# IONIQ6000/av1-go

Measured on AMD Instinct MI355X. Metric: encoded 4K30 frames/sec (whole node) at fixed QP; PSNR-Y delta vs libaom, higher is better.
Workload: dtype u16

## Files before the change

av1-go_amd/csrc/av1_entropy_kernels.hip:

```cpp
#include <stdlib.h>
#include <string.h>
#include <vector>
#include "av1_ops_cdfs.hpp"
#include "av1_ops8.hpp"
#include "av1mi_internal.hpp"
#include "chains_rank.hpp"

namespace av1mi {
using namespace av1ops;

struct Av1EntLaunch {
  FrameView fv;
  int nframes, sbr_n, sbc_n;
  BlockInfo *info;
  op_t *ops; uint32_t ops_cap;
  uint32_t *grouped; uint32_t grouped_cap;
  uint32_t *list_off, *grouped_off;
  uint32_t *cursors;
  uint16_t *slot_total, *slot_base;
  uint16_t *rec;
  uint32_t *nops;
  uint8_t *slots; uint32_t slot_cap;
  uint32_t *tile_size;
  uint64_t *group_sum;
// ... 42 lines not shown
  const long nb = (long)L.fv.w8 * L.fv.h8, i = (long)blockIdx.x * 256 + threadIdx.x;
  if (i >= nb * L.nframes) return;
  const int f = (int)(i / nb), b = (int)(i - (long)f * nb);
  const FrameView v = frame_view<0>(L, f);
  BlockInfo o = {};
  inter_mode_decision(v, b / v.w8, b % v.w8, &o);
  L.info[nb * f + b] = o;
}

struct TileWave {
  template <class T> using Var = LaneVar<T, 1>;
  template <class F> __device__ __forceinline__ void each(F f) { f((int)threadIdx.x); __syncthreads(); }
  __device__ __forceinline__ int scan(Var<int> &v) {
    const int lane = (int)threadIdx.x, x = v.v[0];
    int inc = x;
#pragma unroll
    for (int d = 1; d < 64; d <<= 1) {
      const int y = __shfl_up(inc, d, 64);
      if (lane >= d) inc += y;
    }
    v.v[0] = inc - x;
    return __shfl(inc, 63, 64);
  }
  __device__ __forceinline__ int first(Var<int> &v) { return __shfl(v.v[0], 0, 64); }
  __device__ __forceinline__ uint64_t ballot(Var<int> &v) { return __ballot(v.v[0] != 0); }
};

__global__ __launch_bounds__(64) __attribute__((amdgpu_waves_per_eu(2, 8))) void k_av1_tokens(Av1EntLaunch L) {
  const int tiles = L.sbr_n * L.sbc_n, t = blockIdx.x, f = t / tiles, tt = t - f * tiles, sbr = tt / L.sbc_n, sbc = tt - sbr * L.sbc_n;
  if (sbr < L.sb_rows32) return;
  const FrameView v = frame_view(L, f);
  __shared__ Tile8Mem S;
  const int below = tiles - L.sb_rows32 * L.sbc_n;
  uint16_t *rec = L.rec + ((size_t)f * below + (tt - (tiles - below))) * kBlocksPerTile * kBlockRecords;
  TileWave w;
  PoolAreas out = { L, (size_t)t };
  const int n = tok_tile8(w, S, v, sbr, sbc, rec, L.ops_cap, out);
  if (threadIdx.x == 0) {
    if (n < 0) atomicOr(L.status, 1u);
    L.nops[t] = n < 0 ? 0u : (uint32_t)n;
  }
}

__global__ __launch_bounds__(64) void k_av1_tokens32(Av1EntLaunch L) {
  __shared__ Tile32Mem S;
  const int tiles = L.sbr_n * L.sbc_n, band = L.sb_rows32 * L.sbc_n, f = blockIdx.x / band, tt = blockIdx.x - f * band, sbr = tt / L.sbc_n, sbc = tt - sbr * L.sbc_n;
  const size_t t = (size_t)f * tiles + tt;
  const FrameView v = frame_view<1>(L, f);
  TileWave w;
  PoolAreas out = { L, t };
  const int n = tok_tile32(w, S, v, sbr, sbc, L.ops_cap, out);
  if (threadIdx.x == 0) {
    if (n < 0) atomicOr(L.status, 1u);
    L.nops[t] = n < 0 ? 0u : (uint32_t)n;
  }
}

enum { kChainsInter = 0, kChainsKey8 = 1, kChainsKey32 = 2 };
enum { kChainsCapLds = 0, kChainsCapTickets = 1 };
constexpr int kChainsStaticLds = 64 * 16 * 2, kCuLds = 160 << 10, kChainsXcds = 8, kChainsCusPerXcd = 32;
constexpr int kChainsDefaultCap = kChainsCapTickets, kChainsDefaultWaves = 2;
constexpr int kTicketStride = 32, kTicketRowFirst = kTicketStride, kTicketRowBand32 = kTicketRowFirst + kChainsXcds * kTicketStride;
static unsigned chains_dynamic_lds(int waves) { return waves > 0 && kCuLds / waves > kChainsStaticLds ? (unsigned)(kCuLds / waves - kChainsStaticLds) : 0u; }

__device__ __forceinline__ void chains_item(const Av1EntLaunch &L, int ntiles_all, int flavour, int g, int k, uint16_t *s_big) {
  const int lane = threadIdx.x, t = g * 64 + lane;
  const int sl = (flavour == kChainsInter ? kChainsRankInter : flavour == kChainsKey8 ? kChainsRankKey8 : kChainsRankKey32)[k];
// ... 403 lines not shown
```

av1-go_amd/csrc/av1_ops.hpp:

```cpp
#pragma once
#include <stdint.h>

#if defined(__HIPCC__)
#include <hip/hip_runtime.h>
#define AV1_HD __host__ __device__ inline
#define AV1_UNROLL _Pragma("unroll")
#define AV1_NOUNROLL _Pragma("unroll 1")
#else
#define AV1_HD inline
#define AV1_UNROLL
#define AV1_NOUNROLL
#endif

namespace av1ops {

typedef uint16_t __attribute__((may_alias)) u16a;
typedef uint32_t __attribute__((may_alias)) u32a;
typedef uint64_t __attribute__((may_alias)) u64a;

enum Slot : int {
  S_SKIP = 0,
  S_PART8 = S_SKIP + 3,
  S_PART16 = S_PART8 + 1,
  S_PART32 = S_PART16 + 4,
// ... 46 lines not shown
  if (s == B.eob_y) return B.eob_y_n;
  if (s == B.eob_c) return B.eob_c_n;
  return s < B.base_eob_y ? 2 : s < B.base_y ? 3 : 4;
}
AV1_HD int slot_nsym(int s, bool key) {
  if (const int n = coeff_nsym<kSlots8>(s)) return n;
  if (s < S_PART8) return 2;
  if (s < S_PART16) return 4;
  if (s < S_USE_WIENER) return 10;
  if (s < S_COMMON_END) return 2;
  if (key) {
    if (s < S_UV_MODE) return 13;
    if (s < S_ANGLE) return 14;
    if (s < S_INTRA_TX) return 7;
    return 7;
  }
  if (s < S_MV_JOINT) return 2;
  if (s == S_MV_JOINT) return 4;
  if (s < S_INTER_TX) {
    const int k = (s - S_MV_COMP) & 15;
    return k == MVC_CLASS ? 11 : (k == MVC_CLASS0_FR || k == MVC_CLASS0_FR + 1 || k == MVC_FR) ? 4 : 2;
  }
  return 16;
}
AV1_HD int q_category(int base_q_idx) { return base_q_idx <= 20 ? 0 : base_q_idx <= 60 ? 1 : base_q_idx <= 120 ? 2 : 3; }
AV1_HD int slot_words(int nsym) { return nsym <= 4 ? 4 : nsym <= 8 ? 8 : 16; }

typedef uint32_t op_t;
struct SlotTable { uint16_t off[S_MAX]; uint8_t nsym[(S_MAX + 3) & ~3]; int words; };
AV1_HD op_t op_lit(int n, unsigned v) { return (op_t)(0x80000000u | ((unsigned)n << 27) | (v & 0x7FFu)); }
AV1_HD op_t make_tuple(uint32_t fl, uint32_t fh, int s, int n) { return (op_t)(((unsigned)(n - s) << 19) | ((fl >> 6) << 9) | (fh >> 6)); }
enum { kBlocksPerTile = 64, kSplitHorz = 14, kSplitVert = 15, kListAlign = 4, kBlockRecords = 1024 };

struct Sink {
  uint16_t *rec;
  uint8_t *cnt;
  int zi, nrec, n;
  bool overflow;
  AV1_HD void put(unsigned r) { if (nrec < kBlockRecords) rec[nrec] = (uint16_t)r; else overflow = true; nrec++; n++; }
  AV1_HD void sym(int slot, int s) {
    put(((unsigned)slot << 4) | (unsigned)s);
    uint8_t &c = cnt[slot * kBlocksPerTile + zi];
    if (c == 255) overflow = true; else c++;
  }
  AV1_HD void split(int kind, int slot) { sym(slot, kind ? kSplitVert : kSplitHorz); }
  AV1_HD void lit(unsigned v, int nbits) {
    while (nbits > 11) { nbits -= 11; put(0x8000u | (11u << 11) | ((v >> nbits) & 0x7FFu)); }
    if (nbits > 0) put(0x8000u | ((unsigned)nbits << 11) | (v & ((1u << nbits) - 1u)));
  }
};
struct BlockInfo { uint8_t mode, flags, num, drl; int16_t px, py; };
struct FrameView {
  int w8, h8;
  int key;
  const uint8_t *y_mode, *uv_mode;
  const int16_t *mv;
  const uint8_t *skip;
  const int16_t *lev_y, *lev_u, *lev_v;
  const BlockInfo *info;
  int lr_on[3];
  int8_t lr_unit[2][8];
  int lr_rows[3], lr_cols[3];
  const int8_t *lr_units[3];
  int cdef_bits;
  const uint8_t *cdef_idx;
};
AV1_HD unsigned cdef_index(const FrameView &f, int sbr, int sbc) { return f.cdef_idx ? f.cdef_idx[sbr * ((f.w8 + 7) / 8) + sbc] : 0u; }

AV1_HD int iabs(int v) { return v < 0 ? -v : v; }
AV1_HD int imin(int a, int b) { return a < b ? a : b; }
AV1_HD int imax(int a, int b) { return a > b ? a : b; }
AV1_HD int ilog2(unsigned v) { return 31 - __builtin_clz(v | 1u); }
// ... 543 lines not shown
```

av1-go_amd/csrc/av1_ops8.hpp:

```cpp
#pragma once
#include "av1_ops32.hpp"

namespace av1ops {

enum { kLanes8 = kBlocksPerTile, kReplaySlots = (S_MAX + 1) / 2, kOwn8 = (S_MAX + kLanes8 - 1) / kLanes8 };
static_assert(2 * kReplaySlots >= S_MAX && S_MAX <= 256 && kOwn8 * kLanes8 >= S_MAX && 4 * kLanes8 >= S_MAX, "rows are bytes; two passes cover every slot");

struct Tile8Mem {
  union {
    struct { uint8_t cnt[S_MAX * kBlocksPerTile]; alignas(16) uint8_t mag[kBlocksPerTile * kMagBytes]; } p1;
    uint16_t pos[kReplaySlots * kBlocksPerTile];
  };
  uint16_t total[S_MAX], base[S_MAX];
  uint8_t row[(S_MAX + 3) & ~3];
  uint8_t sums[kBlocksPerTile];
  ScanTables scan;
};
struct SlotCounts8 { uint32_t w[kOwn8][kBlocksPerTile / 4]; };

AV1_HD void replay_block8(const uint16_t *rec, int nrec, uint16_t *pos, const uint8_t *row, int blk, int first, op_t *list, uint32_t *grouped, int row_lo,
                          bool literals) {
  int n = first;
  for (int i0 = 0; i0 < nrec; i0 += 8) {
    struct alignas(16) R8 { uint32_t w[4]; } q = *reinterpret_cast<const R8 *>(rec + i0);
    AV1_UNROLL
    for (int j = 0; j < 8; j++, n++) {
      if (i0 + j >= nrec) break;
      const unsigned r = (q.w[j >> 1] >> (16 * (j & 1))) & 0xFFFFu;
      if (r & 0x8000u) { if (literals) list[n] = op_lit((int)((r >> 11) & 15), r & 0x7FFu); }
      else {
        const unsigned rw = (unsigned)row[r >> 4] - (unsigned)row_lo;
        if (rw < (unsigned)kReplaySlots) { uint16_t &p = pos[rw * kBlocksPerTile + blk]; grouped[p] = ((uint32_t)n << 4) | (r & 15u); p++; }
      }
    }
  }
}

template <class W, class O>
AV1_HD int tok_tile8(W &w, Tile8Mem &S, const FrameView &f, int sbr, int sbc, uint16_t *rec, uint32_t ops_cap, O &out) {
  typedef typename W::template Var<int> LaneInt;
  const int nslots = f.key ? S_KEY_END : S_INTER_END;
  w.each([&](int lane) {
    for (int i = lane; i < S_MAX * kBlocksPerTile / 4; i += kLanes8) reinterpret_cast<u32a *>(S.p1.cnt)[i] = 0;
    if (lane == 0) fill_scan_tables(&S.scan);
    int bx, by;
    demorton8((unsigned)lane, &bx, &by);
    const int r8 = sbr * 8 + by, c8 = sbc * 8 + bx;
    S.sums[by * 8 + bx] = (uint8_t)(r8 < f.h8 && c8 < f.w8 ? block_levels_summary(f, r8 * f.w8 + c8) : 0u);
  });
  int cdef_zi = -1;
  if (f.cdef_bits) {
    if (f.key) cdef_zi = 0;
    else {
      LaneInt coded;
      w.each([&](int lane) {
        int bx, by;
        demorton8((unsigned)lane, &bx, &by);
        const int r8 = sbr * 8 + by, c8 = sbc * 8 + bx;
        coded[lane] = r8 < f.h8 && c8 < f.w8 && !f.skip[r8 * f.w8 + c8];
      });
      const uint64_t m = w.ballot(coded);
      cdef_zi = m ? __builtin_ctzll(m) : -1;
    }
  }
  LaneInt nrec, first;
  w.each([&](int lane) {
    const TokScratch ts = { S.p1.mag + lane * kMagBytes, &S.scan };
    Sink k = { rec + (size_t)lane * kBlockRecords, S.p1.cnt, lane, 0, 0, false };
    tok_block(f, k, ts, sbr, sbc, lane, S.sums, cdef_zi);
    nrec[lane] = k.nrec;
    first[lane] = k.n | (k.overflow ? 1 << 24 : 0);
  });
  const int sum = w.scan(first), words = sum & 0xFFFFFF;
  bool fits = (uint32_t)words <= ops_cap && !(sum >> 24);
  typename W::template Var<SlotCounts8> cnt;
  if (fits) w.each([&](int lane) {
    SlotCounts8 &c = cnt[lane];
    AV1_UNROLL
    for (int q = 0; q < kOwn8; q++) {
      const int sl = lane + kLanes8 * q;
      int tot = 0;
      AV1_UNROLL
      for (int i = 0; i < kBlocksPerTile / 4; i++) {
        const uint32_t u = sl < nslots ? reinterpret_cast<const u32a *>(S.p1.cnt)[sl * (kBlocksPerTile / 4) + i] : 0u;
        c.w[q][i] = u;
#if defined(__HIP_DEVICE_COMPILE__)
        tot = (int)__builtin_amdgcn_sad_u8(u, 0u, (unsigned)tot);
#else
        tot += (int)((u & 0xFF) + ((u >> 8) & 0xFF) + ((u >> 16) & 0xFF) + (u >> 24));
#endif
      }
      if (sl < S_MAX) S.total[sl] = (uint16_t)tot;
    }
  });
  LaneInt ent, used;
  if (fits) w.each([&](int lane) {
    int e = 0, u = 0;
    for (int q = 0; q < 4; q++) {
      const int sl = 4 * lane + q;
      if (sl < nslots) { e += (S.total[sl] + kListAlign - 1) & ~(kListAlign - 1); u += S.total[sl] != 0; }
    }
// ... 14 lines not shown
    for (int q = 0; q < 4; q++) {
      const int sl = 4 * lane + q;
      if (sl >= nslots) break;
      const int tot = S.total[sl];
      S.base[sl] = (uint16_t)run; S.row[sl] = (uint8_t)r;
      run += (tot + kListAlign - 1) & ~(kListAlign - 1); r += tot != 0;
    }
  });
  const int npass = rows <= kReplaySlots ? 1 : 2;
  for (int pass = 0; pass < npass; pass++) {
    const int row_lo = pass * kReplaySlots;
    w.each([&](int lane) {
      const SlotCounts8 &c = cnt[lane];
      AV1_UNROLL
      for (int q = 0; q < kOwn8; q++) {
        const int sl = lane + kLanes8 * q;
        if (sl >= S_MAX) continue;
        if (pass == 0) { const bool on = sl < nslots; out.slot(sl, on ? S.total[sl] : (uint16_t)0, on ? S.base[sl] : (uint16_t)0); }
        if (sl >= nslots || !S.total[sl]) continue;
        const unsigned rw = (unsigned)S.row[sl] - (unsigned)row_lo;
        if (rw >= (unsigned)kReplaySlots) continue;
        int run = S.base[sl];
        AV1_UNROLL
        for (int i = 0; i < kBlocksPerTile / 4; i++) {
          const uint32_t u = c.w[q][i];
          const int p0 = run, p1 = p0 + (int)(u & 0xFF), p2 = p1 + (int)((u >> 8) & 0xFF), p3 = p2 + (int)((u >> 16) & 0xFF);
          run = p3 + (int)(u >> 24);
          u32a *d = reinterpret_cast<u32a *>(S.pos + rw * kBlocksPerTile + 4 * i);
          d[0] = (uint32_t)p0 | ((uint32_t)p1 << 16); d[1] = (uint32_t)p2 | ((uint32_t)p3 << 16);
        }
      }
    });
    w.each([&](int lane) {
      replay_block8(rec + (size_t)lane * kBlockRecords, nrec[lane], S.pos, S.row, lane, first[lane] & 0xFFFFFF, list, grouped, row_lo, pass == 0);
    });
  }
  return words;
}

}
```

av1-go_amd/host/av1_bitstream.hpp:

```cpp
#pragma once
#include <cstddef>
#include <cstdint>
#include <string>
#include <vector>

#include "../../include/av1mi_host.h"

namespace av1mi_host {
namespace av1 {

inline av1mi_colour unspecified_colour() { av1mi_colour c = {}; c.primaries = c.transfer = c.matrix = 2; return c; }
inline bool same_colour(const av1mi_colour &a, const av1mi_colour &b) {
  if (a.primaries != b.primaries || a.transfer != b.transfer || a.matrix != b.matrix || a.full_range != b.full_range || !a.have_mdcv != !b.have_mdcv || !a.have_cll != !b.have_cll) return false;
  if (a.have_cll && (a.max_cll != b.max_cll || a.max_fall != b.max_fall)) return false;
  if (!a.have_mdcv) return true;
  for (int i = 0; i < 3; i++) if (a.primary_x[i] != b.primary_x[i] || a.primary_y[i] != b.primary_y[i]) return false;
  return a.white_x == b.white_x && a.white_y == b.white_y && a.luminance_max == b.luminance_max && a.luminance_min == b.luminance_min;
}
struct SequenceParams {
  int width = 0, height = 0, bit_depth = 8;
  bool film_grain = false;
  av1mi_colour colour = unspecified_colour();
  bool described() const { return colour.primaries != 2 || colour.transfer != 2 || colour.matrix != 2; }
  bool has_colour() const { return described() || colour.full_range || colour.have_mdcv || colour.have_cll; }
  bool operator==(const SequenceParams &o) const {
    return width == o.width && height == o.height && bit_depth == o.bit_depth && film_grain == o.film_grain && same_colour(colour, o.colour);
  }
};
const char *colour_error(const av1mi_colour &c);

inline int visible_width(const av1mi_obu_frame &f) { return f.visible_width ? f.visible_width : f.width; }
inline int visible_height(const av1mi_obu_frame &f) { return f.visible_height ? f.visible_height : f.height; }
inline SequenceParams sequence_params(const av1mi_obu_frame &f) {
  SequenceParams sp; sp.width = visible_width(f); sp.height = visible_height(f); sp.bit_depth = f.bit_depth; sp.film_grain = f.film_grain_present != 0;
  if (f.colour) sp.colour = *f.colour;
  return sp;
}
std::vector<uint8_t> temporal_delimiter_obu();
std::vector<uint8_t> sequence_header_obu(const SequenceParams &sp);
std::vector<uint8_t> metadata_obu_hdr_cll(const av1mi_colour &c);
std::vector<uint8_t> metadata_obu_hdr_mdcv(const av1mi_colour &c);
void append_sequence_obus(const SequenceParams &sp, std::vector<uint8_t> *out);
bool frame_obu(const av1mi_obu_frame &f, int threads, std::vector<uint8_t> *out, std::string *err);
bool frame_obu_from_tiles(const av1mi_obu_frame &f, const uint8_t *payloads, const uint32_t *sizes, int ntiles, std::vector<uint8_t> *out,
                          std::string *err);
std::vector<uint8_t> range_code_raw(const uint32_t *fl, const uint32_t *fh, const uint8_t *sym, const uint8_t *nsym, size_t count);
bool opstream_supported(const av1mi_obu_frame &f, std::string *why);
bool opstream_tiles(const av1mi_obu_frame &f, std::vector<std::vector<uint8_t>> *tiles, std::string *err, int key_rows32 = 0);
int opstream_slots();
int opstream_tile32(const av1mi_obu_frame &f, int sbr, int sbc, uint32_t ops_cap, uint32_t *list, uint32_t *grouped, uint16_t *slot_total, uint16_t *slot_base,
                    std::string *err);
int opstream_tile8(const av1mi_obu_frame &f, int sbr, int sbc, uint32_t ops_cap, uint32_t *list, uint32_t *grouped, uint16_t *slot_total, uint16_t *slot_base,
                   std::string *err);
bool blocks_temporal_unit(const av1mi_obu_blocks &d, bool with_sequence_header, std::vector<uint8_t> *out, std::string *err, int threads = 1,
                          const size_t (*tile_start)[2] = nullptr);
bool temporal_unit(const av1mi_obu_frame &f, bool with_sequence_header, int threads, std::vector<uint8_t> *out, std::string *err);

}
}
```

av1-go_amd/host/av1_opstream.cpp:

```cpp
#include <algorithm>
#include <cstdio>
#include <cstdlib>
#include <cstring>
#include <string>
#include <vector>
#include "../csrc/av1_ops_cdfs.hpp"
#include "../csrc/av1_ops8.hpp"
#include "av1_bitstream.hpp"

namespace av1mi_host {
namespace av1 {

bool opstream_supported(const av1mi_obu_frame &f, std::string *why) {
  auto no = [&](const char *m) { if (why) *why = m; return false; };
  if (f.cdef_bits < 0 || f.cdef_bits > 3) return no("cdef_bits outside 0 .. 3");
  if (f.reduced_tx_set || f.disable_cdf_update) return no("reduced_tx_set / disable_cdf_update must be 0");
  if (f.tile_cols_log2 >= 0 || f.tile_rows_log2 >= 0) return no("one superblock per tile only");
  if (f.angle_y || f.angle_uv || f.cfl_alpha || f.tx_type || f.is_inter) return no("angle deltas, chroma from luma, transform types and intra blocks in inter frames are host-writer only");
  if (f.frame_type == 0 && f.skip) return no("key frames are coded with skip = 0");
  for (int p = 0; p < 3; p++) if (f.lr_type[p] > 1) return no("Wiener restoration only");
  if (f.lr_unit_shift || f.lr_uv_shift) return no("64x64 restoration units only");
  return true;
}

namespace {
bool code_list(std::vector<av1ops::op_t> &list, const std::vector<uint32_t> &grouped, int nslots, const uint16_t *total, const uint16_t *base,
               const av1ops::SlotTable &tab, const uint16_t *image, std::vector<uint8_t> *out, std::string *err) {
  using namespace av1ops;
  const int nops = (int)list.size();
  for (int sl = 0; sl < nslots; sl++)
    if (total[sl]) run_chain(&image[tab.off[sl]], tab.nsym[sl], &grouped[(size_t)base[sl]], total[sl], list.data());
  out->resize((size_t)nops * 2 + 64);
  Coder c;
  uint16_t stage[Coder::kStage];
  c.init(out->data(), (int)out->size(), stage);
  for (int i = 0; i < nops; i++) code_word(c, list[(size_t)i]);
  const int n = c.finish();
  if (n < 0) { if (err) *err = "tile payload overflow"; return false; }
  out->resize((size_t)n);
  return true;
}
struct WaveLoop {
  template <class T> using Var = av1ops::LaneVar<T, av1ops::kLanes32>;
  template <class F> void each(F f) { for (int lane = 0; lane < av1ops::kLanes32; lane++) f(lane); }
  int scan(Var<int> &v) {
    int run = 0;
    for (int lane = 0; lane < av1ops::kLanes32; lane++) { const int x = v.v[lane]; v.v[lane] = run; run += x; }
    return run;
  }
  int first(Var<int> &v) { return v.v[0]; }
  uint64_t ballot(Var<int> &v) {
    uint64_t m = 0;
    for (int lane = 0; lane < av1ops::kLanes32; lane++) m |= (uint64_t)(v.v[lane] != 0) << lane;
    return m;
  }
};
void frame_view_of(const av1mi_obu_frame &f, av1ops::FrameView *v) {
  memset(v, 0, sizeof(*v));
  v->w8 = f.width / 8; v->h8 = f.height / 8; v->key = f.frame_type == 0;
  v->y_mode = f.y_mode; v->uv_mode = f.uv_mode; v->mv = f.mv; v->skip = f.skip; v->lev_y = f.lev_y; v->lev_u = f.lev_u; v->lev_v = f.lev_v;
  v->cdef_bits = f.cdef_bits; v->cdef_idx = f.cdef_bits ? f.cdef_idx : nullptr;
  for (int p = 0; p < 3; p++) {
    v->lr_on[p] = f.lr_type[p] == 1;
    const int ph = p ? (visible_height(f) + 1) >> 1 : visible_height(f), pw = p ? (visible_width(f) + 1) >> 1 : visible_width(f);
    v->lr_rows[p] = std::max((ph + 32) / 64, 1); v->lr_cols[p] = std::max((pw + 32) / 64, 1);
  }
}
bool lr_units_of(const av1mi_obu_frame &f, av1ops::FrameView *v, std::string *err) {
  bool shared = true;
  for (int p = 0; p < 3; p++) {
    if (!v->lr_on[p]) continue;
    const int8_t *u = f.lr_units[p];
    const size_t n = (size_t)v->lr_rows[p] * v->lr_cols[p];
    for (size_t i = 0; i < n; i++) {
      if (u[i * 8] != 0 && u[i * 8] != 1) { if (err) *err = "Wiener restoration units only"; return false; }
      if (memcmp(u, u + i * 8, 8)) shared = false;
    }
    if (p == 2 && v->lr_on[1] && memcmp(u, f.lr_units[1], 8)) shared = false;
  }
  for (int p = 0; p < 3; p++) {
    if (!v->lr_on[p]) continue;
    if (shared) memcpy(v->lr_unit[p ? 1 : 0], f.lr_units[p], 8);
    else v->lr_units[p] = f.lr_units[p];
  }
  return true;
}
}

bool opstream_tiles(const av1mi_obu_frame &f, std::vector<std::vector<uint8_t>> *tiles, std::string *err, int key_rows32) {
  using namespace av1ops;
  if (!opstream_supported(f, err)) return false;
  if (key_rows32 && (f.frame_type != 0 || (key_rows32 & 63) || key_rows32 > f.height || (f.width & 31))) { if (err) *err = "bad 32x32 band"; return false; }
  FrameView v;
  frame_view_of(f, &v);
  std::vector<uint8_t> zskip;
  if (!v.key && !v.skip) { zskip.assign((size_t)v.w8 * v.h8, 0); v.skip = zskip.data(); }
  if (!lr_units_of(f, &v, err)) return false;
  const size_t nb = (size_t)v.w8 * v.h8;
  std::vector<BlockInfo> info(nb);
  v.info = info.data();
  for (size_t b = 0; b < nb; b++) memset(&info[b], 0, sizeof(BlockInfo));
  if (!v.key) for (int r = 0; r < v.h8; r++) for (int c = 0; c < v.w8; c++) inter_mode_decision(v, r, c, &info[(size_t)r * v.w8 + c]);
  const int qcat = q_category(f.base_q_idx);
  SlotTable tab;
  const std::vector<uint16_t> image = default_slot_image(v.key != 0, qcat, &tab);
  const int sbr_n = (v.h8 + 7) / 8, sbc_n = (v.w8 + 7) / 8;
  tiles->assign((size_t)sbr_n * sbc_n, {});
  const int nslots = v.key ? S_KEY_END : S_INTER_END;
  std::vector<Tile8Mem> mem8(1);
  std::vector<uint16_t> rec((size_t)kBlocksPerTile * kBlockRecords);
  const uint32_t ops_cap8 = 1u << 20;
  std::vector<op_t> list8(ops_cap8);
  std::vector<uint32_t> grouped8(65536 + kListAlign);
  const bool stats = getenv("AV1MI_TOK_STATS") != nullptr;
  int st_rec = 0, st_cnt = 0, st_ops = 0, st_over = 0; long st_ops_sum = 0;
  SlotTable tab32;
  const std::vector<uint16_t> image32 = key_rows32 ? default_slot_image_k32(qcat, &tab32) : std::vector<uint16_t>();
  std::vector<Tile32Mem> mem32(key_rows32 ? 1 : 0);
  const uint32_t ops_cap32 = 1u << 20;
  std::vector<op_t> list32(key_rows32 ? ops_cap32 : 0);
  std::vector<uint32_t> grouped32(key_rows32 ? 65536 : 0);
  for (int sbr = 0; sbr < sbr_n; sbr++)
    for (int sbc = 0; sbc < sbc_n; sbc++) {
      if (sbr * 64 < key_rows32) {
        WaveLoop wave;
        uint16_t base[S_MAX], total[S_MAX];
        CallerAreas out = { list32.data(), grouped32.data(), total, base };
        const int words = tok_tile32(wave, mem32[0], v, sbr, sbc, ops_cap32, out);
        if (words < 0) { if (err) *err = "tile too large for 16-bit entry positions"; return false; }
        std::vector<op_t> list(list32.begin(), list32.begin() + words);
        if (!code_list(list, grouped32, K_END, total, base, tab32, image32.data(), &(*tiles)[(size_t)sbr * sbc_n + sbc], err)) return false;
        continue;
      }
      WaveLoop wave;
      uint16_t base[S_MAX], total[S_MAX];
      CallerAreas out = { list8.data(), grouped8.data(), total, base };
      const int words = tok_tile8(wave, mem8[0], v, sbr, sbc, rec.data(), ops_cap8, out);
      if (stats) {
        std::vector<uint8_t> cnt((size_t)S_MAX * kBlocksPerTile, 0);
        const TokScratch ts = { mem8[0].p1.mag, &mem8[0].scan };
        int ops = 0;
        for (int zi = 0; zi < kBlocksPerTile; zi++) {
          Sink k = { rec.data(), cnt.data(), zi, 0, 0, false };
          tok_block(v, k, ts, sbr, sbc, zi, mem8[0].sums, -1);
          st_rec = std::max(st_rec, k.nrec); ops += k.n;
        }
        for (uint8_t c : cnt) st_cnt = std::max(st_cnt, (int)c);
        st_ops = std::max(st_ops, ops); st_ops_sum += ops;
        if (words < 0) { st_over++; continue; }
      }
      if (words < 0) { if (err) *err = "a tile exceeds the tokenizer's capacities (records or symbols of a slot per block, entries per tile)"; return false; }
      std::vector<op_t> list(list8.begin(), list8.begin() + words);
      if (!code_list(list, grouped8, nslots, total, base, tab, image.data(), &(*tiles)[(size_t)sbr * sbc_n + sbc], err)) return false;
    }
  if (stats)
    fprintf(stderr, "[av1mi tok stats] %d tiles: records per block <= %d (capacity %d), symbols of a slot in a block <= %d (255), list words per tile <= %d, mean %.0f; %d tiles over a block capacity\n",
            sbr_n * sbc_n, st_rec, (int)kBlockRecords, st_cnt, st_ops, (double)st_ops_sum / (sbr_n * sbc_n), st_over);
  return true;
}

int opstream_slots() { return av1ops::S_MAX; }

int opstream_tile8(const av1mi_obu_frame &f, int sbr, int sbc, uint32_t ops_cap, uint32_t *list, uint32_t *grouped, uint16_t *slot_total, uint16_t *slot_base,
                   std::string *err) {
  using namespace av1ops;
  if (!opstream_supported(f, err) || sbr < 0 || sbc < 0 || sbr * 64 >= f.height || sbc * 64 >= f.width) return -2;
  FrameView v;
  frame_view_of(f, &v);
  std::vector<uint8_t> zskip;
  if (!v.key && !v.skip) { zskip.assign((size_t)v.w8 * v.h8, 0); v.skip = zskip.data(); }
  if (!lr_units_of(f, &v, err)) return -2;
  std::vector<BlockInfo> info(v.key ? 0 : (size_t)v.w8 * v.h8);
  v.info = info.data();
  if (!v.key) for (int r = 0; r < v.h8; r++) for (int c = 0; c < v.w8; c++) { memset(&info[(size_t)r * v.w8 + c], 0, sizeof(BlockInfo)); inter_mode_decision(v, r, c, &info[(size_t)r * v.w8 + c]); }
  std::vector<Tile8Mem> mem(1);
  std::vector<uint16_t> rec((size_t)kBlocksPerTile * kBlockRecords);
  WaveLoop wave;
  CallerAreas out = { list, grouped, slot_total, slot_base };
  return tok_tile8(wave, mem[0], v, sbr, sbc, rec.data(), ops_cap, out);
}

int opstream_tile32(const av1mi_obu_frame &f, int sbr, int sbc, uint32_t ops_cap, uint32_t *list, uint32_t *grouped, uint16_t *slot_total, uint16_t *slot_base,
                    std::string *err) {
  using namespace av1ops;
  if (!opstream_supported(f, err) || f.frame_type != 0 || (f.width & 31) || sbr < 0 || sbc < 0 || (sbr + 1) * 64 > f.height || sbc * 64 >= f.width) return -2;
  FrameView v;
  frame_view_of(f, &v);
  if (!lr_units_of(f, &v, err)) return -2;
  std::vector<Tile32Mem> mem(1);
  WaveLoop wave;
  CallerAreas out = { list, grouped, slot_total, slot_base };
  return tok_tile32(wave, mem[0], v, sbr, sbc, ops_cap, out);
}

}
}
```

av1-go_amd/host/capi_host.cpp:

```cpp
#include <cstring>
#include "filmgrain.hpp"
#include "daemon.hpp"
#include "av1_bitstream.hpp"
#include "mux.hpp"
#include "y4m.hpp"
#include "backend.hpp"
#include "../csrc/quality.hpp"

using namespace av1mi_host;

static std::vector<std::string> split_lines(const std::string &s) {
  std::vector<std::string> a;
  size_t p = 0, q;
  while ((q = s.find('\n', p)) != std::string::npos) { a.push_back(s.substr(p, q - p)); p = q + 1; }
  a.push_back(s.substr(p));
  return a;
}

extern "C" {
int av1mi_host_determine_quality(int height) { return DetermineQuality(height); }
int av1mi_host_check_size_gate(long long orig, long long neu, double ratio) { return CheckSizeGate(orig, neu, ratio) ? 1 : 0; }
int av1mi_host_transcode_args(const char *in, const char *out, int has_video, int index, int height, int webrip, char *buf, int cap) {
  ProbeResult pr; pr.has_video_stream = has_video != 0; pr.VideoStream.Index = index; pr.VideoStream.Height = height;
  std::vector<std::string> a; std::string err;
// ... 290 lines not shown
  b.insert(b.end(), fr.begin(), fr.end());
  if ((long long)b.size() <= cap && out) memcpy(out, b.data(), b.size());
  return (long long)b.size();
}
long long av1mi_host_opstream_key32_temporal_unit(const av1mi_obu_frame *f, int key_rows32, int with_sequence_header, uint8_t *out, long long cap, char *err,
                                                  int errcap) {
  std::vector<std::vector<uint8_t>> tiles; std::string e;
  auto fail = [&](long long code) { if (err && errcap > 0) { strncpy(err, e.c_str(), errcap - 1); err[errcap - 1] = 0; } return code; };
  if (!av1::opstream_supported(*f, &e)) return fail(-2);
  if (!av1::opstream_tiles(*f, &tiles, &e, key_rows32)) return fail(-1);
  std::vector<uint8_t> cat; std::vector<uint32_t> sizes;
  for (auto &t : tiles) { sizes.push_back((uint32_t)t.size()); cat.insert(cat.end(), t.begin(), t.end()); }
  std::vector<uint8_t> fr;
  if (!av1::frame_obu_from_tiles(*f, cat.data(), sizes.data(), (int)sizes.size(), &fr, &e)) return fail(-1);
  std::vector<uint8_t> b = av1::temporal_delimiter_obu();
  if (with_sequence_header) av1::append_sequence_obus(av1::sequence_params(*f), &b);
  b.insert(b.end(), fr.begin(), fr.end());
  if ((long long)b.size() <= cap && out) memcpy(out, b.data(), b.size());
  return (long long)b.size();
}
int av1mi_host_opstream_slots(void) { return av1::opstream_slots(); }
int av1mi_host_opstream_tile32(const av1mi_obu_frame *f, int sbr, int sbc, uint32_t ops_cap, uint32_t *list, uint32_t *grouped, uint16_t *slot_total,
                               uint16_t *slot_base) {
  if (!f || !list || !grouped || !slot_total || !slot_base) return -2;
  std::string e;
  return av1::opstream_tile32(*f, sbr, sbc, ops_cap, list, grouped, slot_total, slot_base, &e);
}
int av1mi_host_opstream_tile8(const av1mi_obu_frame *f, int sbr, int sbc, uint32_t ops_cap, uint32_t *list, uint32_t *grouped, uint16_t *slot_total,
                              uint16_t *slot_base) {
  if (!f || !list || !grouped || !slot_total || !slot_base) return -2;
  std::string e;
  return av1::opstream_tile8(*f, sbr, sbc, ops_cap, list, grouped, slot_total, slot_base, &e);
}
long long av1mi_host_opstream_temporal_unit(const av1mi_obu_frame *f, int with_sequence_header, uint8_t *out, long long cap, char *err, int errcap) {
  return av1mi_host_opstream_key32_temporal_unit(f, 0, with_sequence_header, out, cap, err, errcap);
}
int av1mi_host_job_json(const char *id, const char *source, const char *status, const char *reason, long long orig, long long neu, char *buf, int cap) {
  Job j; j.ID = id; j.SourcePath = source; j.Status = status; j.Reason = reason; j.OriginalSize = orig; j.NewSize = neu; j.CreatedAt = "2026-01-02T03:04:05Z";
  const std::string s = JobToJSON(j);
  strncpy(buf, s.c_str(), cap - 1); buf[cap - 1] = 0;
  return (int)s.size();
}
double av1mi_host_gpu_usage(int device, const char *sysfs_root) { return GetGPUUsage(device, sysfs_root ? sysfs_root : "/sys"); }
int av1mi_host_mux_units(const char *path, int w, int h, int bd, int fps_n, int fps_d, const uint8_t *data, const long long *sizes,
                         const uint8_t *keys, int n) {
  return av1mi_host_mux_units_colour(path, w, h, bd, fps_n, fps_d, data, sizes, keys, n, nullptr);
}
int av1mi_host_mux_units_display(const char *path, int w, int h, int bd, int fps_n, int fps_d, const uint8_t *data, const long long *sizes,
                                 const uint8_t *keys, int n, int display_w, int display_h) {
  StreamSink sink; std::string err;
  av1::SequenceParams sp; sp.width = w; sp.height = h; sp.bit_depth = bd;
  if (display_w || display_h) sink.set_display_size(display_w, display_h);
  if (!sink.open(path, sp, fps_n, fps_d, &err)) return 1;
  for (int i = 0; i < n; i++) {
    std::vector<uint8_t> tu(data, data + sizes[i]);
    data += sizes[i];
    if (!sink.write(tu, keys[i] != 0, &err)) { sink.abort(); return 2; }
  }
  return sink.close(&err) ? 0 : 3;
}
int av1mi_host_job_pool(const char *sources, int workers, int ngpus, double ratio, const char *state_dir, char *buf, int cap) {
  std::vector<Job> jobs;
  for (const std::string &path : split_lines(sources)) {
    Job j; j.ID = "pool" + std::to_string(jobs.size()); j.SourcePath = path;
    FILE *f = fopen(path.c_str(), "rb");
    if (f) { fseek(f, 0, SEEK_END); j.OriginalSize = ftell(f); fclose(f); }
// ... 13 lines not shown
```

Before: 3482.

## Interleave per-block token records into lane-chunked rows with a compact front region

Replaces the per-block contiguous record buffer (1024 records per block) with a layout where records are stored in 8-record chunks interleaved across the 64 lanes, split into a front region of 12 rows per tile and a tail region stored separately for all tiles. The aim is to make the lanes' writes and the 16-byte replay reads adjacent across the wave, and to keep the commonly used first rows of all tiles packed together so they stay in cache. The cost is extra address arithmetic on every record write and read. Host stats and a self-test check the new layout against the old flat layout.

```diff
diff --git a/av1-go_amd/csrc/av1_entropy_kernels.hip b/av1-go_amd/csrc/av1_entropy_kernels.hip
--- a/av1-go_amd/csrc/av1_entropy_kernels.hip
+++ b/av1-go_amd/csrc/av1_entropy_kernels.hip
@@ -98,7 +98,7 @@
   const FrameView v = frame_view(L, f);
   __shared__ Tile8Mem S;
   const int below = tiles - L.sb_rows32 * L.sbc_n;
-  uint16_t *rec = L.rec + ((size_t)f * below + (tt - (tiles - below))) * kBlocksPerTile * kBlockRecords;
+  const TileRecords rec = TileRecords::of_tile(L.rec, (size_t)f * below + (tt - (tiles - below)), (size_t)L.nframes * below);
   TileWave w;
   PoolAreas out = { L, (size_t)t };
   const int n = tok_tile8(w, S, v, sbr, sbc, rec, L.ops_cap, out);
diff --git a/av1-go_amd/csrc/av1_ops.hpp b/av1-go_amd/csrc/av1_ops.hpp
--- a/av1-go_amd/csrc/av1_ops.hpp
+++ b/av1-go_amd/csrc/av1_ops.hpp
@@ -102,12 +102,28 @@
 AV1_HD op_t make_tuple(uint32_t fl, uint32_t fh, int s, int n) { return (op_t)(((unsigned)(n - s) << 19) | ((fl >> 6) << 9) | (fh >> 6)); }
 enum { kBlocksPerTile = 64, kSplitHorz = 14, kSplitVert = 15, kListAlign = 4, kBlockRecords = 1024 };
 
+enum { kRecChunk = 8, kRecRow = kBlocksPerTile * kRecChunk, kRecRows = kBlockRecords / kRecChunk, kFrontRows = 12, kTailRows = kRecRows - kFrontRows };
+static_assert(kRecRows * kRecChunk == kBlockRecords && kFrontRows > 0 && kFrontRows % 2 == 0 && kTailRows > 0, "whole chunks; a front and a tail");
+#ifdef AV1_TILE_RECORDS_OWN
+AV1_TILE_RECORDS_OWN
+#else
+struct TileRecords {
+  uint16_t *front, *tail;
+  AV1_HD uint16_t *at(int lane, int i) const {
+    const int row = i >> 3;
+    return (row < kFrontRows ? front + row * kRecRow : tail + (row - kFrontRows) * kRecRow) + lane * kRecChunk + (i & (kRecChunk - 1));
+  }
+  static AV1_HD TileRecords of_tile(uint16_t *base, size_t t, size_t tiles) {
+    return { base + t * ((size_t)kFrontRows * kRecRow), base + tiles * ((size_t)kFrontRows * kRecRow) + t * ((size_t)kTailRows * kRecRow) };
+  }
+};
+#endif
 struct Sink {
-  uint16_t *rec;
+  TileRecords rec;
   uint8_t *cnt;
   int zi, nrec, n;
   bool overflow;
-  AV1_HD void put(unsigned r) { if (nrec < kBlockRecords) rec[nrec] = (uint16_t)r; else overflow = true; nrec++; n++; }
+  AV1_HD void put(unsigned r) { if (nrec < kBlockRecords) *rec.at(zi, nrec) = (uint16_t)r; else overflow = true; nrec++; n++; }
   AV1_HD void sym(int slot, int s) {
     put(((unsigned)slot << 4) | (unsigned)s);
     uint8_t &c = cnt[slot * kBlocksPerTile + zi];
diff --git a/av1-go_amd/csrc/av1_ops8.hpp b/av1-go_amd/csrc/av1_ops8.hpp
--- a/av1-go_amd/csrc/av1_ops8.hpp
+++ b/av1-go_amd/csrc/av1_ops8.hpp
@@ -18,11 +18,11 @@
 };
 struct SlotCounts8 { uint32_t w[kOwn8][kBlocksPerTile / 4]; };
 
-AV1_HD void replay_block8(const uint16_t *rec, int nrec, uint16_t *pos, const uint8_t *row, int blk, int first, op_t *list, uint32_t *grouped, int row_lo,
+AV1_HD void replay_block8(const TileRecords &rec, int nrec, uint16_t *pos, const uint8_t *row, int blk, int first, op_t *list, uint32_t *grouped, int row_lo,
                           bool literals) {
   int n = first;
-  for (int i0 = 0; i0 < nrec; i0 += 8) {
-    struct alignas(16) R8 { uint32_t w[4]; } q = *reinterpret_cast<const R8 *>(rec + i0);
+  for (int i0 = 0; i0 < nrec; i0 += kRecChunk) {
+    struct alignas(16) R8 { uint32_t w[4]; } q = *reinterpret_cast<const R8 *>(rec.at(blk, i0));
     AV1_UNROLL
     for (int j = 0; j < 8; j++, n++) {
       if (i0 + j >= nrec) break;
@@ -37,7 +37,7 @@
 }
 
 template <class W, class O>
-AV1_HD int tok_tile8(W &w, Tile8Mem &S, const FrameView &f, int sbr, int sbc, uint16_t *rec, uint32_t ops_cap, O &out) {
+AV1_HD int tok_tile8(W &w, Tile8Mem &S, const FrameView &f, int sbr, int sbc, const TileRecords &rec, uint32_t ops_cap, O &out) {
   typedef typename W::template Var<int> LaneInt;
   const int nslots = f.key ? S_KEY_END : S_INTER_END;
   w.each([&](int lane) {
@@ -66,7 +66,7 @@
   LaneInt nrec, first;
   w.each([&](int lane) {
     const TokScratch ts = { S.p1.mag + lane * kMagBytes, &S.scan };
-    Sink k = { rec + (size_t)lane * kBlockRecords, S.p1.cnt, lane, 0, 0, false };
+    Sink k = { rec, S.p1.cnt, lane, 0, 0, false };
     tok_block(f, k, ts, sbr, sbc, lane, S.sums, cdef_zi);
     nrec[lane] = k.nrec;
     first[lane] = k.n | (k.overflow ? 1 << 24 : 0);
@@ -147,7 +147,7 @@
       }
     });
     w.each([&](int lane) {
-      replay_block8(rec + (size_t)lane * kBlockRecords, nrec[lane], S.pos, S.row, lane, first[lane] & 0xFFFFFF, list, grouped, row_lo, pass == 0);
+      replay_block8(rec, nrec[lane], S.pos, S.row, lane, first[lane] & 0xFFFFFF, list, grouped, row_lo, pass == 0);
     });
   }
   return words;
diff --git a/av1-go_amd/host/av1_bitstream.hpp b/av1-go_amd/host/av1_bitstream.hpp
--- a/av1-go_amd/host/av1_bitstream.hpp
+++ b/av1-go_amd/host/av1_bitstream.hpp
@@ -51,7 +51,7 @@
 int opstream_tile32(const av1mi_obu_frame &f, int sbr, int sbc, uint32_t ops_cap, uint32_t *list, uint32_t *grouped, uint16_t *slot_total, uint16_t *slot_base,
                     std::string *err);
 int opstream_tile8(const av1mi_obu_frame &f, int sbr, int sbc, uint32_t ops_cap, uint32_t *list, uint32_t *grouped, uint16_t *slot_total, uint16_t *slot_base,
-                   std::string *err);
+                   std::string *err, int32_t *block_records = nullptr);
 bool blocks_temporal_unit(const av1mi_obu_blocks &d, bool with_sequence_header, std::vector<uint8_t> *out, std::string *err, int threads = 1,
                           const size_t (*tile_start)[2] = nullptr);
 bool temporal_unit(const av1mi_obu_frame &f, bool with_sequence_header, int threads, std::vector<uint8_t> *out, std::string *err);
diff --git a/av1-go_amd/host/av1_opstream.cpp b/av1-go_amd/host/av1_opstream.cpp
--- a/av1-go_amd/host/av1_opstream.cpp
+++ b/av1-go_amd/host/av1_opstream.cpp
@@ -54,6 +54,10 @@
     for (int lane = 0; lane < av1ops::kLanes32; lane++) m |= (uint64_t)(v.v[lane] != 0) << lane;
     return m;
   }
+};
+struct OneTileRecords {
+  std::vector<uint16_t> front = std::vector<uint16_t>((size_t)av1ops::kFrontRows * av1ops::kRecRow), tail = std::vector<uint16_t>((size_t)av1ops::kTailRows * av1ops::kRecRow);
+  av1ops::TileRecords view() { return { front.data(), tail.data() }; }
 };
 void frame_view_of(const av1mi_obu_frame &f, av1ops::FrameView *v) {
   memset(v, 0, sizeof(*v));
@@ -108,12 +112,13 @@
   tiles->assign((size_t)sbr_n * sbc_n, {});
   const int nslots = v.key ? S_KEY_END : S_INTER_END;
   std::vector<Tile8Mem> mem8(1);
-  std::vector<uint16_t> rec((size_t)kBlocksPerTile * kBlockRecords);
+  OneTileRecords rec;
   const uint32_t ops_cap8 = 1u << 20;
   std::vector<op_t> list8(ops_cap8);
   std::vector<uint32_t> grouped8(65536 + kListAlign);
   const bool stats = getenv("AV1MI_TOK_STATS") != nullptr;
   int st_rec = 0, st_cnt = 0, st_ops = 0, st_over = 0; long st_ops_sum = 0;
+  std::vector<long> st_rows(kRecRows + 2, 0);
   SlotTable tab32;
   const std::vector<uint16_t> image32 = key_rows32 ? default_slot_image_k32(qcat, &tab32) : std::vector<uint16_t>();
   std::vector<Tile32Mem> mem32(key_rows32 ? 1 : 0);
@@ -135,15 +140,19 @@
       WaveLoop wave;
       uint16_t base[S_MAX], total[S_MAX];
       CallerAreas out = { list8.data(), grouped8.data(), total, base };
-      const int words = tok_tile8(wave, mem8[0], v, sbr, sbc, rec.data(), ops_cap8, out);
+      const int words = tok_tile8(wave, mem8[0], v, sbr, sbc, rec.view(), ops_cap8, out);
       if (stats) {
         std::vector<uint8_t> cnt((size_t)S_MAX * kBlocksPerTile, 0);
         const TokScratch ts = { mem8[0].p1.mag, &mem8[0].scan };
         int ops = 0;
         for (int zi = 0; zi < kBlocksPerTile; zi++) {
-          Sink k = { rec.data(), cnt.data(), zi, 0, 0, false };
+          int bx, by;
+          demorton8((unsigned)zi, &bx, &by);
+          if (sbr * 8 + by >= v.h8 || sbc * 8 + bx >= v.w8) continue;
+          Sink k = { rec.view(), cnt.data(), zi, 0, 0, false };
           tok_block(v, k, ts, sbr, sbc, zi, mem8[0].sums, -1);
           st_rec = std::max(st_rec, k.nrec); ops += k.n;
+          st_rows[std::min((k.nrec + kRecChunk - 1) / kRecChunk, (int)kRecRows + 1)]++;
         }
         for (uint8_t c : cnt) st_cnt = std::max(st_cnt, (int)c);
         st_ops = std::max(st_ops, ops); st_ops_sum += ops;
@@ -156,13 +165,18 @@
   if (stats)
     fprintf(stderr, "[av1mi tok stats] %d tiles: records per block <= %d (capacity %d), symbols of a slot in a block <= %d (255), list words per tile <= %d, mean %.0f; %d tiles over a block capacity\n",
             sbr_n * sbc_n, st_rec, (int)kBlockRecords, st_cnt, st_ops, (double)st_ops_sum / (sbr_n * sbc_n), st_over);
+  if (stats) {
+    fprintf(stderr, "[av1mi tok stats] blocks by record rows of %d (front = %d rows):", (int)kRecChunk, (int)kFrontRows);
+    for (size_t r = 0; r < st_rows.size(); r++) if (st_rows[r]) fprintf(stderr, " %zu:%ld", r, st_rows[r]);
+    fprintf(stderr, "\n");
+  }
   return true;
 }
 
 int opstream_slots() { return av1ops::S_MAX; }
 
 int opstream_tile8(const av1mi_obu_frame &f, int sbr, int sbc, uint32_t ops_cap, uint32_t *list, uint32_t *grouped, uint16_t *slot_total, uint16_t *slot_base,
-                   std::string *err) {
+                   std::string *err, int32_t *block_records) {
   using namespace av1ops;
   if (!opstream_supported(f, err) || sbr < 0 || sbc < 0 || sbr * 64 >= f.height || sbc * 64 >= f.width) return -2;
   FrameView v;
@@ -174,10 +188,20 @@
   v.info = info.data();
   if (!v.key) for (int r = 0; r < v.h8; r++) for (int c = 0; c < v.w8; c++) { memset(&info[(size_t)r * v.w8 + c], 0, sizeof(BlockInfo)); inter_mode_decision(v, r, c, &info[(size_t)r * v.w8 + c]); }
   std::vector<Tile8Mem> mem(1);
-  std::vector<uint16_t> rec((size_t)kBlocksPerTile * kBlockRecords);
+  OneTileRecords rec;
   WaveLoop wave;
   CallerAreas out = { list, grouped, slot_total, slot_base };
-  return tok_tile8(wave, mem[0], v, sbr, sbc, rec.data(), ops_cap, out);
+  const int words = tok_tile8(wave, mem[0], v, sbr, sbc, rec.view(), ops_cap, out);
+  if (block_records) {
+    std::vector<uint8_t> cnt((size_t)S_MAX * kBlocksPerTile, 0);
+    const TokScratch ts = { mem[0].p1.mag, &mem[0].scan };
+    for (int zi = 0; zi < kBlocksPerTile; zi++) {
+      Sink k = { rec.view(), cnt.data(), zi, 0, 0, false };
+      tok_block(v, k, ts, sbr, sbc, zi, mem[0].sums, -1);
+      block_records[zi] = k.nrec;
+    }
+  }
+  return words;
 }
 
 int opstream_tile32(const av1mi_obu_frame &f, int sbr, int sbc, uint32_t ops_cap, uint32_t *list, uint32_t *grouped, uint16_t *slot_total, uint16_t *slot_base,
diff --git a/av1-go_amd/host/capi_host.cpp b/av1-go_amd/host/capi_host.cpp
--- a/av1-go_amd/host/capi_host.cpp
+++ b/av1-go_amd/host/capi_host.cpp
@@ -346,6 +346,12 @@
   std::string e;
   return av1::opstream_tile8(*f, sbr, sbc, ops_cap, list, grouped, slot_total, slot_base, &e);
 }
+int av1mi_host_opstream_tile8_records(const av1mi_obu_frame *f, int sbr, int sbc, uint32_t ops_cap, uint32_t *list, uint32_t *grouped, uint16_t *slot_total,
+                                      uint16_t *slot_base, int32_t *block_records) {
+  if (!f || !list || !grouped || !slot_total || !slot_base || !block_records) return -2;
+  std::string e;
+  return av1::opstream_tile8(*f, sbr, sbc, ops_cap, list, grouped, slot_total, slot_base, &e, block_records);
+}
 long long av1mi_host_opstream_temporal_unit(const av1mi_obu_frame *f, int with_sequence_header, uint8_t *out, long long cap, char *err, int errcap) {
   return av1mi_host_opstream_key32_temporal_unit(f, 0, with_sequence_header, out, cap, err, errcap);
 }
diff --git a/av1-go_amd/host/records_selftest.cpp b/av1-go_amd/host/records_selftest.cpp
--- /dev/null
+++ b/av1-go_amd/host/records_selftest.cpp
@@ -0,0 +1,213 @@
+#include <stdint.h>
+#include <stdio.h>
+#include <string.h>
+#include <algorithm>
+#include <string>
+#include <vector>
+#include "av1_bitstream.hpp"
+#define AV1_TILE_RECORDS_OWN \
+  struct TileRecords { uint16_t *base; AV1_HD uint16_t *at(int lane, int i) const { return base + (size_t)lane * kBlockRecords + i; } };
+namespace records_selftest {
+#include "../csrc/av1_ops8.hpp"
+}
+
+namespace {
+namespace ops = records_selftest::av1ops;
+
+struct WaveLoop {
+  template <class T> using Var = ops::LaneVar<T, ops::kLanes32>;
+  template <class F> void each(F f) { for (int lane = 0; lane < ops::kLanes32; lane++) f(lane); }
+  int scan(Var<int> &v) {
+    int run = 0;
+    for (int lane = 0; lane < ops::kLanes32; lane++) { const int x = v.v[lane]; v.v[lane] = run; run += x; }
+    return run;
+  }
+  int first(Var<int> &v) { return v.v[0]; }
+  uint64_t ballot(Var<int> &v) {
+    uint64_t m = 0;
+    for (int lane = 0; lane < ops::kLanes32; lane++) m |= (uint64_t)(v.v[lane] != 0) << lane;
+    return m;
+  }
+};
+
+uint64_t rng_state = 1;
+uint32_t rnd() { rng_state ^= rng_state << 13; rng_state ^= rng_state >> 7; rng_state ^= rng_state << 17; return (uint32_t)(rng_state >> 16); }
+
+struct Frame {
+  int w, h, bd, q; bool key;
+  std::vector<uint8_t> y_mode, uv_mode, skip;
+  std::vector<int16_t> mv, lev_y, lev_u, lev_v;
+  Frame(int w_, int h_, int bd_, int q_, bool key_) : w(w_), h(h_), bd(bd_), q(q_), key(key_) {
+    const size_t nb = (size_t)(w / 8) * (h / 8);
+    y_mode.assign(nb, 0); uv_mode.assign(nb, 0); skip.assign(nb, 0); mv.assign(nb * 2, 0);
+    lev_y.assign(nb * 64, 0); lev_u.assign(nb * 16, 0); lev_v.assign(nb * 16, 0);
+  }
+  av1mi_obu_frame obu() const {
+    av1mi_obu_frame f;
+    memset(&f, 0, sizeof(f));
+    f.width = w; f.height = h; f.bit_depth = bd; f.frame_type = key ? 0 : 1; f.base_q_idx = q;
+    f.tile_cols_log2 = f.tile_rows_log2 = -1;
+    f.lev_y = lev_y.data(); f.lev_u = lev_u.data(); f.lev_v = lev_v.data();
+    if (key) { f.y_mode = y_mode.data(); f.uv_mode = uv_mode.data(); }
+    else { f.mv = mv.data(); f.skip = skip.data(); }
+    return f;
+  }
+  ops::FrameView view(std::vector<ops::BlockInfo> *info) const {
+    ops::FrameView v;
+    memset(&v, 0, sizeof(v));
+    v.w8 = w / 8; v.h8 = h / 8; v.key = key;
+    v.y_mode = y_mode.data(); v.uv_mode = uv_mode.data(); v.mv = mv.data(); v.skip = skip.data();
+    v.lev_y = lev_y.data(); v.lev_u = lev_u.data(); v.lev_v = lev_v.data();
+    for (int p = 0; p < 3; p++) { v.lr_rows[p] = std::max(((p ? (h + 1) / 2 : h) + 32) / 64, 1); v.lr_cols[p] = std::max(((p ? (w + 1) / 2 : w) + 32) / 64, 1); }
+    info->assign((size_t)v.w8 * v.h8, ops::BlockInfo());
+    for (ops::BlockInfo &b : *info) memset(&b, 0, sizeof(b));
+    v.info = info->data();
+    if (!key) for (int r = 0; r < v.h8; r++) for (int c = 0; c < v.w8; c++) ops::inter_mode_decision(v, r, c, &(*info)[(size_t)r * v.w8 + c]);
+    return v;
+  }
+  int block(int sbr, int sbc, int zi) const {
+    int bx, by;
+    ops::demorton8((unsigned)zi, &bx, &by);
+    const int r8 = sbr * 8 + by, c8 = sbc * 8 + bx;
+    return r8 < h / 8 && c8 < w / 8 ? r8 * (w / 8) + c8 : -1;
+  }
+};
+
+void count_records(const Frame &fr, int sbr, int sbc, int nrec[64]) {
+  std::vector<ops::BlockInfo> info;
+  const ops::FrameView v = fr.view(&info);
+  std::vector<ops::Tile8Mem> mem(1);
+  ops::Tile8Mem &S = mem[0];
+  memset(S.p1.cnt, 0, sizeof(S.p1.cnt));
+  ops::fill_scan_tables(&S.scan);
+  for (int zi = 0; zi < 64; zi++) {
+    int bx, by;
+    ops::demorton8((unsigned)zi, &bx, &by);
+    const int b = fr.block(sbr, sbc, zi);
+    S.sums[by * 8 + bx] = (uint8_t)(b >= 0 ? ops::block_levels_summary(v, b) : 0u);
+  }
+  static std::vector<uint16_t> flat((size_t)ops::kBlocksPerTile * ops::kBlockRecords);
+  for (int zi = 0; zi < 64; zi++) {
+    const ops::TokScratch ts = { S.p1.mag, &S.scan };
+    ops::Sink k = { { flat.data() }, S.p1.cnt, zi, 0, 0, false };
+    ops::tok_block(v, k, ts, sbr, sbc, zi, S.sums, -1);
+    nrec[zi] = k.nrec;
+  }
+}
+
+bool shape_block(Frame *fr, int zi, int target) {
+  static const int16_t kValues[] = { 0, 0, 1, -1, 2, 3, -6, 9, 14, -15, 40, -300, 2000, -30000 };
+  const int b = fr->block(0, 0, zi);
+  int nrec[64];
+  count_records(*fr, 0, 0, nrec);
+  for (int it = 0; it < 40000 && nrec[zi] != target; it++) {
+    if (it % 4000 == 3999) {
+      for (int i = 0; i < 64; i++) fr->lev_y[(size_t)b * 64 + i] = 0;
+      for (int i = 0; i < 16; i++) fr->lev_u[(size_t)b * 16 + i] = fr->lev_v[(size_t)b * 16 + i] = 0;
+      count_records(*fr, 0, 0, nrec);
+    }
+    const int p = (int)(rnd() % 96u);
+    int16_t *lev = p < 64 ? &fr->lev_y[(size_t)b * 64 + p] : p < 80 ? &fr->lev_u[(size_t)b * 16 + p - 64] : &fr->lev_v[(size_t)b * 16 + p - 80];
+    const int16_t old = *lev;
+    const int before = nrec[zi] > target ? nrec[zi] - target : target - nrec[zi];
+    *lev = kValues[rnd() % (sizeof(kValues) / sizeof(kValues[0]))];
+    count_records(*fr, 0, 0, nrec);
+    const int after = nrec[zi] > target ? nrec[zi] - target : target - nrec[zi];
+    if (after > before && !(after <= before + 6 && rnd() % 8u == 0)) { *lev = old; count_records(*fr, 0, 0, nrec); }
+  }
+  return nrec[zi] == target;
+}
+
+int failures = 0;
+#define CHECK(cond, ...) do { if (!(cond)) { failures++; fprintf(stderr, "records_selftest: " __VA_ARGS__); fprintf(stderr, "\n"); } } while (0)
+
+int compare_tile(const char *name, const Frame &fr, int sbr, int sbc, uint32_t ops_cap = 1u << 16) {
+  const int ns = ops::S_MAX;
+  const uint32_t fill32 = 0xA5A5A5A5u; const uint16_t fill16 = 0x5A5A;
+  std::vector<uint32_t> list_a(ops_cap, fill32), list_b(ops_cap, fill32), grp_a(ops_cap + 4 * ns, fill32), grp_b(ops_cap + 4 * ns, fill32);
+  std::vector<uint16_t> tot_a(ns, fill16), tot_b(ns, fill16), base_a(ns, fill16), base_b(ns, fill16);
+  const av1mi_obu_frame f = fr.obu();
+  std::string err;
+  const int na = av1mi_host::av1::opstream_tile8(f, sbr, sbc, ops_cap, list_a.data(), grp_a.data(), tot_a.data(), base_a.data(), &err);
+  std::vector<ops::BlockInfo> info;
+  const ops::FrameView v = fr.view(&info);
+  std::vector<ops::Tile8Mem> mem(1);
+  std::vector<uint16_t> flat((size_t)ops::kBlocksPerTile * ops::kBlockRecords);
+  WaveLoop wave;
+  ops::CallerAreas out = { list_b.data(), grp_b.data(), tot_b.data(), base_b.data() };
+  const int nb = ops::tok_tile8(wave, mem[0], v, sbr, sbc, ops::TileRecords{ flat.data() }, ops_cap, out);
+  CHECK(na == nb, "%s tile (%d, %d): %d list words, the plain layout gives %d (%s)", name, sbr, sbc, na, nb, err.c_str());
+  CHECK(list_a == list_b, "%s tile (%d, %d): list words differ", name, sbr, sbc);
+  CHECK(grp_a == grp_b, "%s tile (%d, %d): grouped entries differ", name, sbr, sbc);
+  CHECK(tot_a == tot_b && base_a == base_b, "%s tile (%d, %d): slot totals or bases differ", name, sbr, sbc);
+  if (na < 0) {
+    CHECK(std::all_of(tot_a.begin(), tot_a.end(), [](uint16_t t) { return t == 0; }), "%s: a refused tile keeps a slot total", name);
+    CHECK(std::all_of(list_a.begin(), list_a.end(), [&](uint32_t x) { return x == fill32; }) && std::all_of(grp_a.begin(), grp_a.end(), [&](uint32_t x) { return x == fill32; }),
+          "%s: a refused tile wrote list words or entries", name);
+  }
+  return na;
+}
+
+void noise(Frame *fr, int amplitude, unsigned share_of_256) {
+  auto one = [&](std::vector<int16_t> &lev) { for (int16_t &x : lev) x = rnd() % 256u < share_of_256 ? (int16_t)((int)(rnd() % (2u * amplitude + 1)) - amplitude) : 0; };
+  one(fr->lev_y); one(fr->lev_u); one(fr->lev_v);
+  for (uint8_t &m : fr->y_mode) m = (uint8_t)(rnd() % 13u);
+  for (uint8_t &m : fr->uv_mode) m = (uint8_t)(rnd() % 13u);
+  for (size_t i = 0; i < fr->skip.size(); i++) {
+    fr->skip[i] = rnd() % 4u == 0;
+    fr->mv[2 * i] = (int16_t)(2 * ((int)(rnd() % 41u) - 20)); fr->mv[2 * i + 1] = (int16_t)(2 * ((int)(rnd() % 41u) - 20));
+  }
+}
+}
+
+int main() {
+  const int F = 8 * ops::kFrontRows;
+  for (int key = 1; key >= 0; key--) {
+    Frame fr(64, 64, 8, 60, key != 0);
+    if (!key) for (uint8_t &s : fr.skip) s = 1;
+    {
+      const int b = fr.block(0, 0, 63);
+      if (!key) fr.skip[(size_t)b] = 0;
+      for (int i = 0; i < 64; i++) fr.lev_y[(size_t)b * 64 + i] = -32767;
+      for (int i = 0; i < 16; i++) { fr.lev_u[(size_t)b * 16 + i] = 32767; fr.lev_v[(size_t)b * 16 + i] = -32767; }
+    }
+    int longest[64];
+    count_records(fr, 0, 0, longest);
+    fprintf(stderr, "records_selftest: the longest block leaves %d records (capacity %d)\n", longest[63], (int)ops::kBlockRecords);
+    CHECK(longest[63] > 8 * (ops::kRecRows - 16) && longest[63] <= ops::kBlockRecords, "the longest block: %d records", longest[63]);
+    const int targets[] = { F - 1, F, F + 1, 2 * F + 5, 8 * 64 - 1, 8 * 100 };
+    const int blocks[] = { 20, 21, 22, 40, 61, 62 };
+    for (size_t i = 0; i < sizeof(targets) / sizeof(targets[0]); i++) {
+      if (!key) fr.skip[(size_t)fr.block(0, 0, blocks[i])] = 0;
+      CHECK(shape_block(&fr, blocks[i], targets[i]), "no block of %d records found (%s)", targets[i], key ? "key" : "inter");
+    }
+    int nrec[64];
+    count_records(fr, 0, 0, nrec);
+    fprintf(stderr, "records_selftest: %s tile, records per block:", key ? "key" : "inter");
+    for (int zi = 0; zi < 64; zi++) fprintf(stderr, " %d", nrec[zi]);
+    fprintf(stderr, "\n");
+    for (int want : { 7, 8, 9 })
+      if (key) CHECK(std::find(nrec, nrec + 64, want) != nrec + 64, "no block of %d records in the key tile", want);
+    const int words = compare_tile(key ? "boundaries, key" : "boundaries, inter", fr, 0, 0);
+    CHECK(words > 0, "the tile of boundary counts was refused");
+    CHECK(compare_tile("one word over the list's capacity", fr, 0, 0, (uint32_t)words - 1) == -1, "a tile over the list's capacity was not refused");
+    CHECK(compare_tile("exactly the list's capacity", fr, 0, 0, (uint32_t)words) == words, "a tile of exactly the list's capacity was refused");
+  }
+  const struct { int amplitude; unsigned share; } kNoise[] = { { 2, 20 }, { 40, 200 }, { 30000, 256 } };
+  for (int key = 1; key >= 0; key--)
+    for (const auto &nz : kNoise)
+      for (int bd = 8; bd <= 10; bd += 2) {
+        Frame fr(136, 72, bd, nz.amplitude > 100 ? 1 : 128, key != 0);
+        noise(&fr, nz.amplitude, nz.share);
+        for (int sbr = 0; sbr < 2; sbr++) for (int sbc = 0; sbc < 3; sbc++) {
+          const int n = compare_tile("noise", fr, sbr, sbc, 1u << 17);
+          CHECK(n > 0, "a tile of noise was refused");
+        }
+        int edge[64];
+        count_records(fr, 1, 2, edge);
+        CHECK(edge[0] > 0 && std::count(edge, edge + 64, 0) == 63, "the corner tile's blocks outside the frame leave records");
+      }
+  if (failures) { fprintf(stderr, "records_selftest: %d FAILURES\n", failures); return 1; }
+  printf("records_selftest OK (front %d rows, tail %d rows of %d records per lane)\n", (int)ops::kFrontRows, (int)ops::kTailRows, (int)ops::kRecChunk);
+  return 0;
+}
```

Result: no change. 3468 (-0.4%).
